# daniestevez/gr4-packet-modem

Hardware: AMD Instinct MI355X
Metric: RX Msamples/s (syncword-detect + RRC chain) (higher is better)
Workload: dtype f32; 1 GPU; configs[1]: 1 channel/GPU, full RX front end (SyncwordDetection 9 bins FFT 2048 + tag gate + CFC + 32-arm RRC SymbolFilter + wipe-off + Costas) on resident burst+AWGN stream; channels_per_gpu=1, freq_bins=9, parallelism=channel-per-gpu x1, input=generated on each GPU, pipelined_streams=4, pipeline_driver=native (gr4pm_packet_receiver), windows=2, correlator_lookahead=2

## Files before the change

### gr4-packet-modem_amd/_abi.py

```python
import ctypes as C
import os

import numpy as np

_HERE = os.path.dirname(os.path.abspath(__file__))
LIB_PATH = os.environ.get("GR4PM_LIB") or os.path.join(_HERE, "libgr4pm_hip.so")

OK = 0
INSUFFICIENT_INPUT_ITEMS = 1
INSUFFICIENT_OUTPUT_ITEMS = 2
TAG_SYNCWORD = 1
TAG_OTHER = 2

TAG_DTYPE = np.dtype(
    [
        ("index", "<u8"),
        ("amplitude", "<f4"),
        ("phase", "<f4"),
        ("freq", "<f8"),
        ("freq_bin", "<i4"),
        ("noise_power", "<f4"),
        ("esn0_db", "<f4"),
        ("time_est", "<f4"),
        ("flags", "<i4"),
# ... 298 lines not shown
    "gr4pm_iq_unpack", "gr4pm_iq_pack",
    "gr4pm_ddc_taps", "gr4pm_ddc_create", "gr4pm_ddc_destroy", "gr4pm_ddc_reset", "gr4pm_ddc_output_items",
    "gr4pm_ddc_frequencies", "gr4pm_ddc_process", "gr4pm_ddc_process_iq",
    "gr4pm_ddc_rational_taps", "gr4pm_ddc_create_rational", "gr4pm_ddc_extract", "gr4pm_ddc_extract_iq",
    "gr4pm_duc_taps", "gr4pm_duc_create", "gr4pm_duc_destroy", "gr4pm_duc_reset", "gr4pm_duc_output_items",
    "gr4pm_duc_frequencies", "gr4pm_duc_process",
    "gr4pm_duc_rational_taps", "gr4pm_duc_create_rational",
    "gr4pm_spectrum_window", "gr4pm_spectrum_float_run", "gr4pm_spectrum_create", "gr4pm_spectrum_destroy",
    "gr4pm_spectrum_reset", "gr4pm_spectrum_process", "gr4pm_spectrum_process_iq", "gr4pm_spectrum_read",
    "gr4pm_find_carriers",
    "gr4pm_spectrogram_create", "gr4pm_spectrogram_destroy", "gr4pm_spectrogram_reset", "gr4pm_spectrogram_rows",
    "gr4pm_spectrogram_process", "gr4pm_spectrogram_process_iq", "gr4pm_spectrogram_band_power", "gr4pm_find_bursts",
    "gr4pm_line_spectrum_float_run", "gr4pm_line_spectrum_create", "gr4pm_line_spectrum_destroy", "gr4pm_line_spectrum_process",
    "gr4pm_find_line", "gr4pm_simplest_ratio",
    "gr4pm_row_resampler_taps", "gr4pm_row_resampler_create", "gr4pm_row_resampler_destroy",
    "gr4pm_row_resampler_output_lengths", "gr4pm_row_resampler_tile_items", "gr4pm_row_resampler_process",
]

_lib = None


class Gr4pmError(RuntimeError):
    """what the reference raises as gr::exception"""


def lib():
    global _lib
    if _lib is not None:
        return _lib
    if not os.path.exists(LIB_PATH):
        raise ImportError(
            f"{LIB_PATH} is missing: build it with `python -c 'import __graft_entry__ as g; g.build()'` "
            "(hipcc --offload-arch=gfx950). There is no CPU fallback.")
    try:
        import torch
    except ImportError:
        pass
    L = C.CDLL(LIB_PATH)
    vp, sz, szp = C.c_void_p, C.c_size_t, C.POINTER(C.c_size_t)
    L.gr4pm_last_error.restype = C.c_char_p
    L.gr4pm_version.restype = C.c_char_p
    L.gr4pm_device_count.restype = C.c_int
    if hasattr(L, "gr4pm_test_fail_allocations"):
        L.gr4pm_test_fail_allocations.argtypes = [C.c_long, C.c_long]
        L.gr4pm_test_fail_allocations.restype = None
        L.gr4pm_test_allocation_count.restype = C.c_ulonglong
    L.gr4pm_syncword_detection_create.argtypes = [C.POINTER(SyncwordDetectionParams), C.POINTER(vp)]
    L.gr4pm_syncword_detection_destroy.argtypes = [vp]
    L.gr4pm_syncword_detection_destroy.restype = None
    L.gr4pm_syncword_detection_reset.argtypes = [vp]
    L.gr4pm_syncword_detection_syncword_samples_size.argtypes = [vp]
    L.gr4pm_syncword_detection_syncword_samples_size.restype = sz
    L.gr4pm_syncword_detection_self_corr.argtypes = [vp]
    L.gr4pm_syncword_detection_self_corr.restype = C.c_float
    L.gr4pm_syncword_detection_items_consumed.argtypes = [vp]
    L.gr4pm_syncword_detection_items_consumed.restype = C.c_uint64
    L.gr4pm_syncword_detection_scan_counts.argtypes = [vp, sz, C.POINTER(C.c_uint64), C.POINTER(C.c_uint64)]
    L.gr4pm_syncword_detection_scan_counts.restype = None
    L.gr4pm_syncword_detection_process.argtypes = [vp, vp, sz, sz, vp, sz, szp, vp, sz, vp]
    L.gr4pm_syncword_detection_last_zpow.argtypes = [vp, vp, sz]
    L.gr4pm_syncword_detection_correlate_only.argtypes = [vp, vp, sz, sz]
    L.gr4pm_syncword_detection_hint_next.argtypes = [vp, vp, sz, sz]
    L.gr4pm_syncword_detection_announce.argtypes = [vp, vp, sz, sz]
    L.gr4pm_syncword_detection_filter_create.argtypes = [C.POINTER(SdfParams), C.POINTER(vp)]
    L.gr4pm_syncword_detection_filter_destroy.argtypes = [vp]
    L.gr4pm_syncword_detection_filter_destroy.restype = None
    L.gr4pm_syncword_detection_filter_reset.argtypes = [vp]
    L.gr4pm_syncword_detection_filter_process.argtypes = [vp, vp, sz, vp, sz, C.c_int, vp, sz, sz, szp, szp, szp,
                                                          C.POINTER(C.c_int)]
    L.gr4pm_syncword_detection_filter_gate.argtypes = [vp, vp, sz, vp, sz, C.c_int, vp, szp]
    L.gr4pm_rotator_create.argtypes = [C.POINTER(RotatorParams), C.POINTER(vp)]
    L.gr4pm_rotator_destroy.argtypes = [vp]
    L.gr4pm_rotator_destroy.restype = None
    L.gr4pm_rotator_reset.argtypes = [vp]
    L.gr4pm_rotator_process.argtypes = [vp, vp, sz, sz, vp, vp, vp, sz]
    L.gr4pm_costas_loop_create.argtypes = [C.POINTER(CostasParams), C.POINTER(vp)]
    L.gr4pm_costas_loop_destroy.argtypes = [vp]
    L.gr4pm_costas_loop_destroy.restype = None
    L.gr4pm_costas_loop_reset.argtypes = [vp]
    L.gr4pm_costas_loop_coeffs.argtypes = [vp, C.POINTER(C.c_float), C.POINTER(C.c_float)]
    L.gr4pm_costas_loop_coeffs.restype = None
    L.gr4pm_costas_loop_set.argtypes = [vp, C.c_double, C.c_int]
    L.gr4pm_costas_loop_process.argtypes = [vp, vp, sz, sz, vp, vp, vp, sz]
    L.gr4pm_syncword_wipeoff_create.argtypes = [C.POINTER(WipeoffParams), C.POINTER(vp)]
    L.gr4pm_syncword_wipeoff_destroy.argtypes = [vp]
    L.gr4pm_syncword_wipeoff_destroy.restype = None
    L.gr4pm_syncword_wipeoff_reset.argtypes = [vp]
    L.gr4pm_syncword_wipeoff_process.argtypes = [vp, vp, sz, vp, vp, sz]
    L.gr4pm_syncword_wipeoff_process_channels.argtypes = [vp, sz, vp, sz, vp, vp, vp]
    L.gr4pm_cfc_symbol_filter_run_channels.argtypes = [vp, C.c_int, vp, sz, vp, sz, sz, vp, sz, vp, vp, vp, sz, vp, vp, vp, sz, sz]
    L.gr4pm_multichannel_receiver_set_input_in_place.argtypes = [vp, C.c_int]
    L.gr4pm_interp_fir_create.argtypes = [C.POINTER(InterpFirParams), C.POINTER(vp)]
    L.gr4pm_interp_fir_destroy.argtypes = [vp]
    L.gr4pm_interp_fir_destroy.restype = None
    L.gr4pm_interp_fir_reset.argtypes = [vp]
    L.gr4pm_interp_fir_process.argtypes = [vp, vp, sz, vp]
    L.gr4pm_symbol_filter_create.argtypes = [C.POINTER(SymbolFilterParams), C.POINTER(vp)]
    L.gr4pm_symbol_filter_destroy.argtypes = [vp]
    L.gr4pm_symbol_filter_destroy.restype = None
    L.gr4pm_symbol_filter_reset.argtypes = [vp]
    L.gr4pm_symbol_filter_process.argtypes = [vp, vp, sz, vp, sz, vp, sz, vp, sz, szp, szp, szp]
    L.gr4pm_cfc_symbol_filter_process.argtypes = [vp, vp, vp, sz, vp, sz, vp, sz, vp, sz, szp, szp, szp]
    L.gr4pm_cfc_symbol_filter_plan.argtypes = [vp, sz, vp, sz, C.POINTER(C.c_int)]
    L.gr4pm_cfc_symbol_filter_run.argtypes = [vp, C.c_int, vp, vp, sz, vp, sz, vp, sz, vp, sz, szp, szp, szp]
    L.gr4pm_pfb_arb_resampler_create.argtypes = [C.POINTER(PfbArbParams), C.POINTER(vp)]
    L.gr4pm_pfb_arb_resampler_destroy.argtypes = [vp]
    L.gr4pm_pfb_arb_resampler_destroy.restype = None
    L.gr4pm_pfb_arb_resampler_reset.argtypes = [vp]
    L.gr4pm_pfb_arb_resampler_process.argtypes = [vp, vp, sz, vp, sz, szp, szp]
    L.gr4pm_payload_metadata_insert_create.argtypes = [C.POINTER(PmiParams), C.POINTER(vp)]
    L.gr4pm_payload_metadata_insert_destroy.argtypes = [vp]
    L.gr4pm_payload_metadata_insert_destroy.restype = None
    L.gr4pm_payload_metadata_insert_reset.argtypes = [vp]
    L.gr4pm_payload_metadata_insert_process.argtypes = [vp, vp, sz, vp, sz, vp, sz, vp, sz, C.c_int, vp, sz,
                                                        szp, szp, szp, szp, szp]
    L.gr4pm_costas_loop_process_packets.argtypes = [vp, vp, sz, vp, vp, sz]
    L.gr4pm_syncword_detection_filter_gate_resolve.argtypes = [vp, vp]
    L.gr4pm_payload_metadata_insert_resolve.argtypes = [vp, vp]
    L.gr4pm_syncword_remove_create.argtypes = [C.POINTER(SyncwordRemoveParams), C.POINTER(vp)]
    L.gr4pm_syncword_remove_destroy.argtypes = [vp]
    L.gr4pm_syncword_remove_destroy.restype = None
    L.gr4pm_syncword_remove_reset.argtypes = [vp]
    L.gr4pm_syncword_remove_process.argtypes = [vp, vp, sz, vp, vp, sz, vp, sz, szp, szp]
    L.gr4pm_constellation_llr_decoder_create.argtypes = [C.POINTER(LlrParams), C.POINTER(vp)]
    L.gr4pm_constellation_llr_decoder_destroy.argtypes = [vp]
    L.gr4pm_constellation_llr_decoder_destroy.restype = None
    L.gr4pm_constellation_llr_decoder_process.argtypes = [vp, vp, sz, vp, sz, vp, sz, vp, sz, szp, szp]
    L.gr4pm_additive_scrambler_create.argtypes = [C.POINTER(ScramblerParams), C.POINTER(vp)]
    L.gr4pm_additive_scrambler_destroy.argtypes = [vp]
    L.gr4pm_additive_scrambler_destroy.restype = None
    L.gr4pm_additive_scrambler_reset.argtypes = [vp]
    L.gr4pm_additive_scrambler_process.argtypes = [vp, vp, sz, vp, vp, sz]
    L.gr4pm_header_payload_split_create.argtypes = [C.POINTER(HeaderPayloadSplitParams), C.POINTER(vp)]
    L.gr4pm_header_payload_split_destroy.argtypes = [vp]
    L.gr4pm_header_payload_split_destroy.restype = None
    L.gr4pm_header_payload_split_reset.argtypes = [vp]
    L.gr4pm_header_payload_split_process.argtypes = [vp, vp, sz, vp, szp, vp, szp, vp, sz, vp, szp, vp, szp, sz]
    L.gr4pm_header_payload_split_process_c64.argtypes = [vp, vp, sz, vp, szp, vp, szp, vp, sz, vp, szp, vp, szp, sz]
    L.gr4pm_header_fec_decoder_create.argtypes = [C.POINTER(HeaderFecDecoderParams), C.POINTER(vp)]
    L.gr4pm_header_fec_decoder_destroy.argtypes = [vp]
    L.gr4pm_header_fec_decoder_destroy.restype = None
    L.gr4pm_header_fec_decoder_process.argtypes = [vp, vp, sz, vp, vp]
    L.gr4pm_header_parse.argtypes = [vp, vp, sz, vp, vp]
    L.gr4pm_header_parse.restype = None
    L.gr4pm_binary_slicer_process.argtypes = [vp, sz, vp, C.c_int, vp]
    L.gr4pm_pack_bits_process.argtypes = [vp, sz, vp, sz, C.c_uint, C.c_int, vp]
    L.gr4pm_slice_pack_process.argtypes = [vp, sz, vp, vp]
    L.gr4pm_crc_check_create.argtypes = [C.POINTER(CrcCheckParams), C.POINTER(vp)]
    L.gr4pm_crc_check_destroy.argtypes = [vp]
    L.gr4pm_crc_check_destroy.restype = None
    L.gr4pm_crc_check_compute.argtypes = [vp, vp, sz]
    L.gr4pm_crc_check_compute.restype = C.c_uint64
    L.gr4pm_crc_check_process.argtypes = [vp, vp, vp, vp, sz, vp, vp, szp]
    L.gr4pm_mapper_process.argtypes = [vp, sz, vp, vp, sz, C.c_int, vp]
    L.gr4pm_burst_shaper_process.argtypes = [vp, sz, vp, C.c_int, vp, sz, vp, sz, vp, vp, sz, vp]
    L.gr4pm_packet_receiver_create.argtypes = [C.POINTER(PacketReceiverParams), C.POINTER(vp)]
    L.gr4pm_packet_receiver_destroy.argtypes = [vp]
    L.gr4pm_packet_receiver_destroy.restype = None
    L.gr4pm_packet_receiver_submit.argtypes = [vp, vp, sz, vp, vp, sz, C.c_uint64, vp, sz, vp, sz, vp, sz]
    L.gr4pm_packet_receiver_announce.argtypes = [vp, vp, sz]
    L.gr4pm_multichannel_receiver_create.argtypes = [C.POINTER(MultiChannelReceiverParams), C.POINTER(vp)]
    L.gr4pm_multichannel_receiver_destroy.argtypes = [vp]
    L.gr4pm_multichannel_receiver_destroy.restype = None
    L.gr4pm_multichannel_receiver_announce.argtypes = [vp, vp, sz, sz]
    L.gr4pm_multichannel_receiver_process.argtypes = [vp, vp, sz, sz, C.c_uint64, vp, sz, szp, szp, vp, szp, vp, szp]
    L.gr4pm_multichannel_receiver_submit.argtypes = [vp, vp, sz, sz, C.c_uint64, vp, sz, szp]
# ... 115 lines not shown
```

### gr4-packet-modem_amd/csrc/costas_loop.hip

```cpp
#include "stream_blocks.hpp"
#include "hostlogic/costas_plan.hpp"

namespace gr4pm {
namespace {

struct CostasState {
    float phase, freq;
};
using hostlogic::CostasSeg;

__device__ __forceinline__ void sincosf_glibc(float y, float* s_out, float* c_out)
{
    const double hpi_inv = 0x1.45F306DC9C883p+23, hpi = 0x1.921FB54442D18p0;
    const double C0 = 0x1p0, C1 = -0x1.ffffffd0c621cp-2, C2 = 0x1.55553e1068f19p-5, C3 = -0x1.6c087e89a359dp-10,
                 C4 = 0x1.99343027bf8c3p-16, S1 = -0x1.555545995a603p-3, S2 = 0x1.1107605230bc4p-7,
                 S3 = -0x1.994eb3774cf24p-13;
    const double x0 = static_cast<double>(y);
    const int n = (static_cast<int>(x0 * hpi_inv) + 0x800000) >> 24;
    const double x = fma(-static_cast<double>(n), hpi, x0);
    const double x2 = x * x;
    const double x3 = x * x2;
    const double s1 = fma(x2, S3, S2);
    const double x7 = x3 * x2;
    const double sp = fma(x7, s1, fma(x3, S1, x));
    const double x4 = x2 * x2;
    const double c2 = fma(x2, C4, C3);
    const double c1 = fma(x2, C1, C0);
    const double x6 = x4 * x2;
    const double cp = fma(x6, c2, fma(x4, C2, c1));
    float sn = static_cast<float>(sp), cs = static_cast<float>(cp);
    const unsigned sb = __builtin_amdgcn_bitop3_b32(0x7fffffffu, __float_as_uint(sn), static_cast<unsigned>(__double2hiint(x)), 0xca);
    const unsigned cb = __float_as_uint(cs);
    const unsigned swap = static_cast<unsigned>(__builtin_amdgcn_sbfe(n, 0, 1));
    const unsigned s0 = __builtin_amdgcn_bitop3_b32(swap, cb, sb, 0xca);
    const unsigned c0 = __builtin_amdgcn_bitop3_b32(swap, sb, cb, 0xca);
    const unsigned q = static_cast<unsigned>(n) << 30;
    *s_out = __uint_as_float(__builtin_amdgcn_bitop3_b32(s0, q, 0x80000000u, 0x78));
    *c_out = __uint_as_float(__builtin_amdgcn_bitop3_b32(c0, q + 0x40000000u, 0x80000000u, 0x78));
}

__device__ __forceinline__ float costas_wrap(float phase, float pi_f)
{
    const float K = 0x1p100f, two_pi = 2.0f * pi_f;
    const float pi_below = __uint_as_float(__float_as_uint(pi_f) - 1u);
    float up, down;
    asm("v_fma_f32 %0, %2, %3, -%4 clamp\n\t"
        "v_fma_f32 %1, -%2, %3, -%5 clamp"
        : "=&v"(up), "=&v"(down)
        : "v"(phase), "v"(K), "v"(pi_below * K), "v"(pi_f * K));
    return __builtin_fmaf(up - down, -two_pi, phase);
}

template <int CONSTELLATION>
__device__ __forceinline__ cf costas_step(cf x, float& phase, float& freq, float k1, float k2)
{
    const float pi_f = 3.14159265358979323846f;
    float sn, cs;
#ifdef GR4PM_COSTAS_HW_SINCOS
    sn = __sinf(phase);
    cs = __cosf(phase);
#else
    sincosf_glibc(phase, &sn, &cs);
#endif
    const cf lo = { cs, -sn };
    const cf z = cmul(x, lo);
    float error;
    if constexpr (CONSTELLATION == 0) error = z.y;
    else if constexpr (CONSTELLATION == 1) error = z.x * z.y;
    else error = (z.x > 0 ? z.y : -z.y) + (z.y > 0 ? -z.x : z.x);
    freq += k2 * error;
    phase += k1 * error + freq;
    phase = costas_wrap(phase, pi_f);
    return z;
}

template <int CONSTELLATION, int KV = 8>
__device__ __forceinline__ void costas_run(const cf* __restrict__ in, cf* __restrict__ out, size_t base,
                                           unsigned len, float& phase, float& freq, float k1, float k2)
{
    auto step = [&](cf x) -> cf { return costas_step<CONSTELLATION>(x, phase, freq, k1, k2); };
    constexpr int kV = KV;
    constexpr unsigned kC = 2 * kV;
    unsigned j = 0;
    if (((base + j) & 1) && j < len) {
        out[base + j] = step(in[base + j]);
        ++j;
    }
    const unsigned n_chunks = (len - j) / kC;
    if (n_chunks > 0) {
        const float4* ip = reinterpret_cast<const float4*>(in + base + j);
        float4* op = reinterpret_cast<float4*>(out + base + j);
        float4 a[kV], b[kV];
        auto load = [&](float4(&v)[kV], unsigned c) {
            const float4* p = ip + static_cast<size_t>(min(c, n_chunks - 1)) * kV;
#pragma unroll
            for (int u = 0; u < kV; ++u) v[u] = p[u];
            asm volatile("" : "+v"(phase), "+v"(freq) : : "memory");
        };
        auto run = [&](float4(&v)[kV], unsigned c) {
#pragma unroll
            for (int u = 0; u < kV; ++u) {
                const cf z0 = step(cf{ v[u].x, v[u].y });
                const cf z1 = step(cf{ v[u].z, v[u].w });
                v[u] = make_float4(z0.x, z0.y, z1.x, z1.y);
            }
            float4* q = op + static_cast<size_t>(c) * kV;
#pragma unroll
            for (int u = 0; u < kV; ++u) q[u] = v[u];
        };
        load(a, 0);
        unsigned c = 0;
        for (; c + 2 <= n_chunks; c += 2) {
            load(b, c + 1);
            run(a, c);
            load(a, c + 2);
            run(b, c + 1);
        }
        if (c < n_chunks) run(a, c);
        j += n_chunks * kC;
    }
    for (; j < len; ++j) out[base + j] = step(in[base + j]);
}

template <int CONSTELLATION, int KV = 8>
__global__ void k_costas(const CostasSeg* __restrict__ segs, unsigned n_segs,
                         const CostasState* __restrict__ state, CostasState* __restrict__ state_next,
                         float k1, float k2,
                         const cf* __restrict__ in, cf* __restrict__ out, size_t stride)
{
    const unsigned s = blockIdx.x * blockDim.x + threadIdx.x;
    if (s >= n_segs) return;
    __builtin_amdgcn_s_setprio(GR4PM_SERIAL_PRIO);
    const CostasSeg g = segs[s];
    float phase, freq;
    if (g.mode == 0) {
        phase = state[g.channel].phase;
        freq = state[g.channel].freq;
    } else {
        phase = g.phase0;
        freq = 0.0f;
    }
    costas_run<CONSTELLATION, KV>(in, out, static_cast<size_t>(g.channel) * stride + g.start, g.len, phase, freq, k1,
                              k2);
    if (g.last) {
        state_next[g.channel].phase = phase;
        state_next[g.channel].freq = freq;
    }
}

template <int CONSTELLATION, int KV>
__global__ __attribute__((amdgpu_num_vgpr(16))) void k_costas_cap(const CostasSeg* __restrict__ segs, unsigned n_segs,
                                                               const CostasState* __restrict__ state,
                                                               CostasState* __restrict__ state_next, float k1, float k2,
                                                               const cf* __restrict__ in, cf* __restrict__ out,
                                                               size_t stride)
{
    const unsigned s = blockIdx.x * blockDim.x + threadIdx.x;
    if (s >= n_segs) return;
    __builtin_amdgcn_s_setprio(GR4PM_SERIAL_PRIO);
    const CostasSeg g = segs[s];
    float phase, freq;
    if (g.mode == 0) {
        phase = state[g.channel].phase;
        freq = state[g.channel].freq;
    } else {
        phase = g.phase0;
        freq = 0.0f;
    }
    costas_run<CONSTELLATION, KV>(in, out, static_cast<size_t>(g.channel) * stride + g.start, g.len, phase, freq, k1, k2);
    if (g.last) {
        state_next[g.channel].phase = phase;
        state_next[g.channel].freq = freq;
    }
}

using hostlogic::CostasChain;
using hostlogic::CostasPiece;
template <int KV>
__device__ __forceinline__ void costas_chains_body(const CostasChain* __restrict__ chains, unsigned n_chains,
                                                   const CostasPiece* __restrict__ pieces,
                                                   const CostasState* __restrict__ state,
                                                   CostasState* __restrict__ state_next, const cf* __restrict__ in,
                                                   cf* __restrict__ out)
{
    const unsigned s = blockIdx.x * blockDim.x + threadIdx.x;
    if (s >= n_chains) return;
    __builtin_amdgcn_s_setprio(GR4PM_SERIAL_PRIO);
    const CostasChain ch = chains[s];
    float phase, freq;
    if (ch.mode == 0) {
        phase = state[0].phase;
        freq = state[0].freq;
    } else {
        phase = ch.phase0;
        freq = 0.0f;
    }
    for (unsigned q = 0; q < ch.n_pieces; ++q) {
        const CostasPiece pc = pieces[ch.piece0 + q];
        const cf* src = in + pc.in_off;
        if (pc.constellation == 0) costas_run<0, KV>(src, out, pc.start, pc.len, phase, freq, pc.k1, pc.k2);
        else if (pc.constellation == 1) costas_run<1, KV>(src, out, pc.start, pc.len, phase, freq, pc.k1, pc.k2);
        else costas_run<2, KV>(src, out, pc.start, pc.len, phase, freq, pc.k1, pc.k2);
    }
    if (ch.last) {
        state_next[0].phase = phase;
        state_next[0].freq = freq;
    }
}
template <int KV>
__global__ void k_costas_chains(const CostasChain* __restrict__ chains, unsigned n_chains,
                                const CostasPiece* __restrict__ pieces, const CostasState* __restrict__ state,
                                CostasState* __restrict__ state_next, const cf* __restrict__ in,
                                cf* __restrict__ out)
{
    costas_chains_body<KV>(chains, n_chains, pieces, state, state_next, in, out);
}
__global__ __attribute__((amdgpu_num_vgpr(16))) void k_costas_chains_cap(const CostasChain* __restrict__ chains, unsigned n_chains,
                                                                      const CostasPiece* __restrict__ pieces,
                                                                      const CostasState* __restrict__ state,
                                                                      CostasState* __restrict__ state_next,
                                                                      const cf* __restrict__ in, cf* __restrict__ out)
{
    costas_chains_body<2>(chains, n_chains, pieces, state, state_next, in, out);
}

__global__ void k_sincosf(const float* __restrict__ x, size_t n, float* __restrict__ sn, float* __restrict__ cs)
{
    const size_t i = static_cast<size_t>(blockIdx.x) * blockDim.x + threadIdx.x;
    if (i < n) sincosf_glibc(x[i], sn + i, cs + i);
}

__global__ void k_costas_wrap(const float* __restrict__ x, size_t n, float* __restrict__ out)
{
    const size_t i = static_cast<size_t>(blockIdx.x) * blockDim.x + threadIdx.x;
    if (i < n) out[i] = costas_wrap(x[i], 3.14159265358979323846f);
}

#ifdef GR4PM_EXPERIMENTS
__global__ __launch_bounds__(64) void k_serial_fake(unsigned ticks, float* sink)
{
    const unsigned long long t0 = wall_clock64();
    float x = threadIdx.x;
    while (wall_clock64() - t0 < ticks) {
#pragma unroll
        for (int i = 0; i < 32; ++i) x = __builtin_fmaf(x, 1.0001f, 0.5f);
    }
    if (x == 12345.0f) *sink = x;
}
#endif

}
}

using namespace gr4pm;

struct gr4pm_costas_loop : gr4pm::hostlogic::CostasHostState {
    size_t n_channels;
    hipStream_t stream;
    DevBuf<CostasState> state;
    int st_cur = 0;
    int small_footprint = 0;
    DevBuf<CostasSeg> segs;
    DevBuf<CostasChain> chains;
    DevBuf<CostasPiece> pieces;
};
using hostlogic::costas_coeffs;

extern "C" {

gr4pm_status gr4pm_costas_loop_create(const gr4pm_costas_loop_params* p, gr4pm_costas_loop** out)
try {
    if (!p || !out || p->n_channels == 0 || p->constellation < 0 || p->constellation > 2)
        return GR4PM_ERR_INVALID;
    *out = nullptr;
    GR4PM_TRY(require_device());
    std::unique_ptr<gr4pm_costas_loop> h(new (std::nothrow) gr4pm_costas_loop);
    if (!h) return GR4PM_ERR_NOMEM;
    h->loop_bandwidth = p->loop_bandwidth;
    h->constellation = p->constellation;
    h->n_channels = p->n_channels;
    h->stream = static_cast<hipStream_t>(p->stream);
    costas_coeffs(*h);
    GR4PM_TRY(h->state.alloc(2 * h->n_channels));
    GR4PM_TRY(h->state.zero(h->stream));
    static const char* form = gr4pm::experiment_env("GR4PM_COSTAS_FORM", false);
    if (form) h->small_footprint = std::min(2, std::max(0, atoi(form)));
    return finish_create(h, out, "costas_loop");
}
GR4PM_ABI_CATCH
void gr4pm_costas_loop_destroy(gr4pm_costas_loop* h)
try {
    if (!h) return;
    (void)hipStreamSynchronize(h->stream);
    delete h;
}
GR4PM_ABI_CATCH_VOID
gr4pm_status gr4pm_costas_loop_reset(gr4pm_costas_loop* h)
try {
    if (!h) return GR4PM_ERR_INVALID;
    GR4PM_TRY(h->state.zero(h->stream));
    GR4PM_HIP_TRY(hipStreamSynchronize(h->stream));
    h->st_cur = 0;
    return GR4PM_OK;
}
GR4PM_ABI_CATCH
void gr4pm_costas_loop_coeffs(const gr4pm_costas_loop* h, float* k1, float* k2)
try {
    *k1 = h->k1;
    *k2 = h->k2;
}
GR4PM_ABI_CATCH_VOID
gr4pm_status gr4pm_costas_loop_set(gr4pm_costas_loop* h, double loop_bandwidth, int constellation)
try {
    if (!h || constellation < 0 || constellation > 2) return GR4PM_ERR_INVALID;
    h->loop_bandwidth = loop_bandwidth;
    h->constellation = constellation;
    costas_coeffs(*h);
    return GR4PM_OK;
}
GR4PM_ABI_CATCH

extern "C++" {
template <typename NOf>
static gr4pm_status costas_process_impl(gr4pm_costas_loop* h, const gr4pm_c64* in, size_t stride, NOf n_of,
                                        gr4pm_c64* out, const gr4pm_tag* tags, const uint32_t* tag_channel,
                                        size_t n_tags)
{
    static const bool costas_no_sort = gr4pm::experiment_env("GR4PM_COSTAS_NO_SORT", false) != nullptr;
    std::vector<CostasSeg> segs;
    hostlogic::costas_segments(h->n_channels, n_of, tags, tag_channel, n_tags, costas_no_sort, segs);
    hipStream_t s = h->stream;
    GR4PM_TRY(upload_vec(h->segs, segs, s));
    if (timing_skip("seg_stats")) {
        size_t longest = 0, total = 0;
        for (const auto& g : segs) longest = std::max<size_t>(longest, g.len), total += g.len;
        fprintf(stderr, "[gr4pm costas] %zu segments, %zu items, longest %zu\n", segs.size(), total, longest);
    }
    static const unsigned wg = gr4pm::experiment_env_wg("GR4PM_COSTAS_WG", 64u, 1u, 1024u);
    const dim3 grid(grid_for(segs.size(), wg)), block(wg);
    const unsigned n_segs = static_cast<unsigned>(segs.size());
    const CostasState* st_in = h->state.p + h->st_cur * h->n_channels;
    CostasState* st_out = h->state.p + (h->st_cur ^ 1) * h->n_channels;
    h->st_cur ^= 1;
    auto launch = [&](auto kernel) {
#ifdef GR4PM_EXPERIMENTS
        if (timing_skip("costas_fake")) {
            unsigned wgs = grid.x, ticks = 83000u, lds = 0u;
            static const char* fake = gr4pm::experiment_env("GR4PM_FAKE", true);
            if (fake) sscanf(fake, "%u,%u,%u", &wgs, &ticks, &lds);
            wgs = std::max(wgs, 1u);
            if (lds > 48 * 1024)
                (void)hipFuncSetAttribute(reinterpret_cast<const void*>(k_serial_fake),
                                          hipFuncAttributeMaxDynamicSharedMemorySize, static_cast<int>(lds));
            hipLaunchKernelGGL(k_serial_fake, dim3(wgs), block, lds, s, ticks, reinterpret_cast<float*>(st_out));
            return;
        }
#endif
        if (timing_skip("costas")) return;
        hipLaunchKernelGGL(kernel, grid, block, 0, s, h->segs.p, n_segs, st_in, st_out, h->k1, h->k2,
                           reinterpret_cast<const cf*>(in), reinterpret_cast<cf*>(out), stride);
    };
    size_t call_symbols = 0;
    for (const auto& g : segs) call_symbols += g.len;
    static const char* cap_min = gr4pm::experiment_env("GR4PM_COSTAS_CAP_MIN_LOG2", false);
    const size_t cap_from = size_t{ 1 } << (cap_min ? std::min(40, std::max(0, atoi(cap_min))) : 25);
    if (h->small_footprint >= 2 && call_symbols >= cap_from) {
        if (h->constellation == 0) launch(k_costas_cap<0, 2>);
        else if (h->constellation == 1) launch(k_costas_cap<1, 2>);
        else launch(k_costas_cap<2, 2>);
    } else if (h->small_footprint == 1) {
        if (h->constellation == 0) launch(k_costas<0, 2>);
        else if (h->constellation == 1) launch(k_costas<1, 2>);
        else launch(k_costas<2, 2>);
    } else {
        if (h->constellation == 0) launch(k_costas<0, 8>);
        else if (h->constellation == 1) launch(k_costas<1, 8>);
        else launch(k_costas<2, 8>);
    }
    GR4PM_HIP_TRY(hipGetLastError());
    GR4PM_HIP_TRY(final_sync(s));
    return GR4PM_OK;
}
}

gr4pm_status gr4pm_costas_loop_set_small_footprint(gr4pm_costas_loop* h, int on)
try {
    if (!h) return GR4PM_ERR_INVALID;
    h->small_footprint = on < 0 ? 0 : (on > 2 ? 2 : on);
    return GR4PM_OK;
}
GR4PM_ABI_CATCH

gr4pm_status gr4pm_costas_loop_process(gr4pm_costas_loop* h, const gr4pm_c64* in, size_t stride, size_t n,
                                       gr4pm_c64* out, const gr4pm_tag* tags, const uint32_t* tag_channel,
                                       size_t n_tags)
try {
    if (!h) return GR4PM_ERR_INVALID;
    if (n == 0) return GR4PM_OK;
    if (!in || !out) {
        set_error("null sample pointer");
        return GR4PM_ERR_INVALID;
    }
    return costas_process_impl(h, in, stride, [n](size_t) { return n; }, out, tags, tag_channel, n_tags);
}
GR4PM_ABI_CATCH

gr4pm_status gr4pm_costas_loop_process_ragged(gr4pm_costas_loop* h, const gr4pm_c64* in, size_t stride,
                                              const size_t* n_per_channel, gr4pm_c64* out, const gr4pm_tag* tags,
                                              const uint32_t* tag_channel, size_t n_tags)
try {
    if (!h || !n_per_channel) return GR4PM_ERR_INVALID;
    if (!in || !out) {
        set_error("null sample pointer");
        return GR4PM_ERR_INVALID;
    }
    return costas_process_impl(h, in, stride, [n_per_channel](size_t c) { return n_per_channel[c]; }, out, tags,
                               tag_channel, n_tags);
}
GR4PM_ABI_CATCH

gr4pm_status gr4pm_costas_loop_process_packets(gr4pm_costas_loop* h, const gr4pm_c64* in, size_t n,
                                               gr4pm_c64* out, const gr4pm_packet_tag* tags, size_t n_tags)
try {
    return gr4pm::costas_loop_process_packets_from(h, in, nullptr, 0, n, out, tags, n_tags);
}
GR4PM_ABI_CATCH

}

gr4pm_status gr4pm::costas_loop_process_packets_from(gr4pm_costas_loop* h, const gr4pm_c64* in, const hostlogic::CopySpan* spans,
                                                     size_t n_spans, size_t n, gr4pm_c64* out, const gr4pm_packet_tag* tags,
                                                     size_t n_tags)
{
    if (!h) return GR4PM_ERR_INVALID;
    if (h->n_channels != 1) {
        set_error("process_packets needs a single-channel CostasLoop");
        return GR4PM_ERR_INVALID;
    }
    if (n == 0) return GR4PM_OK;
    if (!in || !out) {
        set_error("null sample pointer");
        return GR4PM_ERR_INVALID;
    }
    std::vector<CostasChain> chains;
    std::vector<CostasPiece> pieces;
    GR4PM_TRY(hostlogic::costas_packet_chains(*h, spans, n_spans, n, tags, n_tags, chains, pieces));
    if (chains.empty()) return GR4PM_OK;
    hipStream_t s = h->stream;
    GR4PM_TRY(upload_vec(h->chains, chains, s));
    GR4PM_TRY(upload_vec(h->pieces, pieces, s));
    if (!timing_skip("costas_chains")) {
        static const char* cap_min = gr4pm::experiment_env("GR4PM_COSTAS_CAP_MIN_LOG2", false);
        const size_t cap_from = size_t{ 1 } << (cap_min ? std::min(40, std::max(0, atoi(cap_min))) : 25);
        auto launch = [&](auto kernel) {
            hipLaunchKernelGGL(kernel, dim3(grid_for(chains.size(), 64)), dim3(64), 0, s, h->chains.p,
                               static_cast<unsigned>(chains.size()), h->pieces.p, h->state.p + h->st_cur,
                               h->state.p + (h->st_cur ^ 1), reinterpret_cast<const cf*>(in), reinterpret_cast<cf*>(out));
        };
        if (h->small_footprint >= 2 && n >= cap_from) launch(k_costas_chains_cap);
        else if (h->small_footprint == 1) launch(k_costas_chains<2>);
        else launch(k_costas_chains<8>);
    }
    h->st_cur ^= 1;
    GR4PM_HIP_TRY(hipGetLastError());
    GR4PM_HIP_TRY(final_sync(s));
    return GR4PM_OK;
}

extern "C" {

gr4pm_status gr4pm_sincosf(const float* x, size_t n, float* sin_out, float* cos_out)
// ... 26 lines not shown
```

### gr4-packet-modem_amd/csrc/multichannel_receiver.hip

```cpp
#include <algorithm>
#include <chrono>
#include <cmath>
#include <cstdio>
#include <cstdlib>
#include <condition_variable>
#include <cstring>
#include <deque>
#include <memory>
#include <mutex>
#include <thread>
#include <vector>

#include "common.hpp"
#include "hostlogic/slot_queue.hpp"

using namespace gr4pm;

constexpr int kMcSlots = 4;

struct gr4pm_multichannel_receiver {
    gr4pm_multichannel_receiver_params p{};
    int device = 0;
    gr4pm_syncword_detection* sd = nullptr;
    hipStream_t sd_stream = nullptr;
// ... 237 lines not shown
            s.status = exception_status(which == 1 ? "multichannel receiver, stage 1"
                                                   : which == 2 ? "multichannel receiver, stage 2" : "multichannel receiver, stage 3");
            std::strncpy(s.error, gr4pm_last_error(), sizeof(s.error) - 1);
            if (which == 3) s.t_done = std::chrono::steady_clock::now();
        });
}

extern "C" {

gr4pm_status gr4pm_multichannel_receiver_create(const gr4pm_multichannel_receiver_params* p,
                                                gr4pm_multichannel_receiver** out)
try {
    if (!p || !out || p->n_channels == 0 || p->samples_per_symbol == 0 || p->max_items < 2048) return GR4PM_ERR_INVALID;
    *out = nullptr;
    GR4PM_TRY(require_device());
    auto* h = new (std::nothrow) gr4pm_multichannel_receiver;
    if (!h) return GR4PM_ERR_NOMEM;
    h->p = *p;
    h->p.tags_cap = std::max<size_t>(p->tags_cap, 64);
    auto bail = [&](gr4pm_status st) {
        gr4pm_multichannel_receiver_destroy(h);
        return st;
    };
    const unsigned n_workers = static_cast<unsigned>(std::min<size_t>(std::max(p->workers, 1), p->n_channels));
    int least = 0, greatest = 0;
    if (hipDeviceGetStreamPriorityRange(&least, &greatest) != hipSuccess) return bail(GR4PM_ERR_HIP);
    if (hipStreamCreateWithPriority(&h->sd_stream, hipStreamNonBlocking, greatest) != hipSuccess) return bail(GR4PM_ERR_HIP);
    h->streams.assign(n_workers, nullptr);
    for (unsigned w = 0; w < n_workers; ++w) {
        const int prio = w % 3 == 0 ? 0 : (w % 3 == 1 ? greatest : least);
        if (hipStreamCreateWithPriority(&h->streams[w], hipStreamNonBlocking, prio) != hipSuccess) return bail(GR4PM_ERR_HIP);
    }
    const size_t sps = p->samples_per_symbol;
    std::vector<float> rrc(((sps * 11) | 1));
    const size_t n_rrc = gr4pm_firdes_root_raised_cosine(1.0, static_cast<double>(sps), 1.0, 0.35, sps * 11, rrc.data());
    if (n_rrc == 0) return bail(GR4PM_ERR_NOMEM);
    rrc.resize(n_rrc);
    float norm = 0.0f;
    for (float v : rrc) norm += v * v;
    norm = std::sqrt(norm);
    for (float& v : rrc) v /= norm;
    static const uint8_t syncword[64] = {
        0, 0, 0, 0, 0, 0, 1, 1, 0, 1, 0, 0, 0, 1, 1, 1, 0, 1, 1, 1, 0, 1, 1, 0, 1, 1, 0, 0, 0, 1, 1, 1,
        0, 0, 1, 0, 0, 1, 1, 1, 0, 0, 1, 0, 1, 0, 0, 0, 1, 0, 0, 1, 0, 1, 0, 1, 1, 0, 1, 1, 0, 0, 0, 0 };
    const gr4pm_c64 bpsk[2] = { { 1.0f, 0.0f }, { -1.0f, 0.0f } };
    gr4pm_syncword_detection_params sp{};
    sp.fft_size = 2048;
    sp.samples_per_symbol = sps;
    sp.rrc_taps = rrc.data();
    sp.n_rrc_taps = rrc.size();
    sp.syncword = syncword;
    sp.n_syncword = 64;
    sp.constellation = bpsk;
    sp.n_constellation = 2;
    sp.min_freq_bin = -p->syncword_freq_bins;
    sp.max_freq_bin = p->syncword_freq_bins;
    sp.time_threshold = 768;
    sp.power_threshold = p->syncword_threshold;
    sp.n_channels = p->n_channels;
    sp.max_items = p->max_items;
    sp.stream = h->sd_stream;
    gr4pm_status st = gr4pm_syncword_detection_create(&sp, &h->sd);
    if (st != GR4PM_OK) return bail(st);
    gr4pm::sd_set_coresident(h->sd, true);
    const size_t arms = 32;
    std::vector<float> pfb(((arms * sps * 11) | 1));
    const size_t n_pfb = gr4pm_firdes_root_raised_cosine(static_cast<double>(arms) / static_cast<double>(norm),
                                                         static_cast<double>(arms * sps), 1.0, 0.35, arms * sps * 11,
                                                         pfb.data());
    if (n_pfb == 0) return bail(GR4PM_ERR_NOMEM);
    pfb.resize(n_pfb - 1);
    float bipolar[64];
    for (int i = 0; i < 64; ++i) bipolar[i] = syncword[i] ? -1.0f : 1.0f;
    h->chains.reset(new (std::nothrow) gr4pm_multichannel_receiver::Chain[p->n_channels]);
    if (!h->chains) return bail(GR4PM_ERR_NOMEM);
    if (hipStreamCreateWithPriority(&h->batch_stream, hipStreamNonBlocking, greatest) != hipSuccess) return bail(GR4PM_ERR_HIP);
    gr4pm_rotator_params rp{ 1, 0.0f, (rrc.size() - 1) / 2 + sps, p->n_channels, h->batch_stream };
    if ((st = gr4pm_rotator_create(&rp, &h->cfc)) != GR4PM_OK) return bail(st);
    if (hipStreamCreateWithPriority(&h->costas_stream, hipStreamNonBlocking, least) != hipSuccess) return bail(GR4PM_ERR_HIP);
    gr4pm_costas_loop_params cp{ 0.01, p->costas_constellation, p->n_channels, h->costas_stream };
    if ((st = gr4pm_costas_loop_create(&cp, &h->costas)) != GR4PM_OK) return bail(st);
    {
        static const char* small = gr4pm::experiment_env("GR4PM_COSTAS_SMALL", false);
        if (small) (void)gr4pm_costas_loop_set_small_footprint(h->costas, atoi(small));
    }
    for (size_t c = 0; c < p->n_channels; ++c) {
        auto& ch = h->chains[c];
        hipStream_t s = h->streams[c % n_workers];
        gr4pm_syncword_detection_filter_params fp{ sps, 64, 128, s };
        if ((st = gr4pm_syncword_detection_filter_create(&fp, &ch.sdf)) != GR4PM_OK) return bail(st);
        gr4pm_symbol_filter_params fsp{ sps, pfb.data(), pfb.size(), arms, rrc.size() - 1, 0, s };
        if ((st = gr4pm_symbol_filter_create(&fsp, &ch.symf)) != GR4PM_OK) return bail(st);
        gr4pm_syncword_wipeoff_params wp{ bipolar, 64, s };
        if ((st = gr4pm_syncword_wipeoff_create(&wp, &ch.wipe)) != GR4PM_OK) return bail(st);
    }
    {
        const char* e = getenv("GR4PM_MC_PER_CHANNEL");
        h->per_channel_launches = e && e[0] == '1';
        const size_t C = p->n_channels;
        h->v_symf.resize(C);
        h->v_wipe.resize(C);
        for (size_t c = 0; c < C; ++c) {
            h->v_symf[c] = h->chains[c].symf;
            h->v_wipe[c] = h->chains[c].wipe;
        }
        h->v_tags_in.assign(C, nullptr);
        h->v_tags_out.assign(C, nullptr);
        h->v_n_tags_in.assign(C, 0);
        h->v_n_tags_out.assign(C, 0);
        h->v_produced.assign(C, 0);
    }
    h->hist = 2 * 768 + 1;
    h->sd_fft = sp.fft_size;
    h->sd_stride = sp.fft_size - (63 * sps + rrc.size()) + 1;
    for (auto& t : h->tails) {
        if ((st = t.alloc(h->hist * p->n_channels)) != GR4PM_OK) return bail(st);
        if ((st = t.zero(h->sd_stream)) != GR4PM_OK) return bail(st);
    }
    if (hipStreamSynchronize(h->sd_stream) != hipSuccess) return bail(GR4PM_ERR_HIP);
    h->y_stride = (p->max_items + 63) & ~size_t{ 63 };
    for (auto& sl : h->slots) {
        if ((st = sl.y.alloc(h->y_stride * p->n_channels)) != GR4PM_OK) return bail(st);
        sl.det_tags.resize(p->n_channels * h->p.tags_cap);
        sl.n_det.assign(p->n_channels, 0);
        sl.produced.assign(p->n_channels, 0);
        sl.ch.resize(p->n_channels);
        for (auto& cb : sl.ch) {
            cb.tags.resize(h->p.tags_cap);
            cb.sym_tags.resize(h->p.tags_cap + 64);
        }
    }
    if (hipGetDevice(&h->device) != hipSuccess) return bail(GR4PM_ERR_HIP);
    try {
        h->workers.reserve(n_workers);
        for (unsigned w = 0; w < n_workers; ++w) h->workers.emplace_back([h, w] { h->worker(w); });
        h->t_stage1 = std::thread([h] { h->stage_loop(1); });
        h->t_stage2 = std::thread([h] { h->stage_loop(2); });
        h->t_stage3 = std::thread([h] { h->stage_loop(3); });
    } catch (...) {
        return bail(exception_status("gr4pm_multichannel_receiver_create (threads)"));
    }
    *out = h;
    return GR4PM_OK;
}
GR4PM_ABI_CATCH

void gr4pm_multichannel_receiver_destroy(gr4pm_multichannel_receiver* h)
try {
    if (!h) return;
    {
        std::lock_guard<std::mutex> l(h->m);
        h->quit = true;
    }
    h->cv_go.notify_all();
    h->to_stage1.stop();
    h->to_stage2.stop();
    h->to_stage3.stop();
    h->done.stop();
    for (std::thread* t : { &h->t_stage1, &h->t_stage2, &h->t_stage3 })
        if (t->joinable()) t->join();
    for (auto& t : h->workers)
        if (t.joinable()) t.join();
    gr4pm_syncword_detection_destroy(h->sd);
    for (size_t c = 0; h->chains && c < h->p.n_channels; ++c) {
        auto& ch = h->chains[c];
        gr4pm_syncword_detection_filter_destroy(ch.sdf);
        gr4pm_symbol_filter_destroy(ch.symf);
// ... 156 lines not shown
```

Measured before the change: 67550 Msamples/s.

## Add LDS ring-buffered async-load Costas kernel and make it the receiver default

Adds a Costas loop kernel in which each lane streams its segment through an 8-slot LDS ring filled with global_load_lds_dwordx4 direct-to-LDS loads. Several chunks are kept in flight so the serial per-symbol phase recursion no longer stalls on global memory latency. The multichannel receiver now sets small_footprint=2 by default, which picks the ring kernel when the wavefront fits within the CU count and the call is large enough. Other changes: the wrap constants move to SGPR operands, VGPRs are capped at 16, and an unaligned head or tail symbol is handled separately. The risks are extra LDS usage, tight register pressure, and a default switch of kernel path for large calls.

```diff
diff --git a/gr4-packet-modem_amd/_abi.py b/gr4-packet-modem_amd/_abi.py
--- a/gr4-packet-modem_amd/_abi.py
+++ b/gr4-packet-modem_amd/_abi.py
@@ -404,6 +404,8 @@
     L.gr4pm_costas_loop_coeffs.restype = None
     L.gr4pm_costas_loop_set.argtypes = [vp, C.c_double, C.c_int]
     L.gr4pm_costas_loop_process.argtypes = [vp, vp, sz, sz, vp, vp, vp, sz]
+    L.gr4pm_costas_loop_process_ragged.argtypes = [vp, vp, sz, szp, vp, vp, vp, sz]
+    L.gr4pm_costas_loop_set_small_footprint.argtypes = [vp, C.c_int]
     L.gr4pm_syncword_wipeoff_create.argtypes = [C.POINTER(WipeoffParams), C.POINTER(vp)]
     L.gr4pm_syncword_wipeoff_destroy.argtypes = [vp]
     L.gr4pm_syncword_wipeoff_destroy.restype = None
diff --git a/gr4-packet-modem_amd/csrc/costas_loop.hip b/gr4-packet-modem_amd/csrc/costas_loop.hip
--- a/gr4-packet-modem_amd/csrc/costas_loop.hip
+++ b/gr4-packet-modem_amd/csrc/costas_loop.hip
@@ -1,5 +1,6 @@
 #include "stream_blocks.hpp"
 #include "hostlogic/costas_plan.hpp"
+#include "hostlogic/costas_ring_plan.hpp"
 
 namespace gr4pm {
 namespace {
@@ -47,7 +48,7 @@
     asm("v_fma_f32 %0, %2, %3, -%4 clamp\n\t"
         "v_fma_f32 %1, -%2, %3, -%5 clamp"
         : "=&v"(up), "=&v"(down)
-        : "v"(phase), "v"(K), "v"(pi_below * K), "v"(pi_f * K));
+        : "v"(phase), "v"(K), "s"(pi_below * K), "s"(pi_f * K));
     return __builtin_fmaf(up - down, -two_pi, phase);
 }
 
@@ -174,6 +175,88 @@
     }
 }
 
+__device__ __forceinline__ void ring_dma(const float4* src, uint32_t slot_base)
+{
+    asm volatile("s_mov_b32 m0, %1\n\ts_nop 0\n\tglobal_load_lds_dwordx4 %0, off" : : "v"(src), "s"(slot_base) : "memory");
+}
+template <unsigned VMCNT>
+__device__ __forceinline__ void ring_wait()
+{
+    asm volatile("s_waitcnt vmcnt(%c0) lgkmcnt(0)" : : "i"(VMCNT) : "memory");
+}
+
+template <int CONSTELLATION>
+__global__ __attribute__((amdgpu_num_vgpr(16))) void k_costas_ring(
+    const CostasSeg* __restrict__ segs, unsigned n_segs, const CostasState* __restrict__ state,
+    CostasState* __restrict__ state_next, float k1, float k2, const cf* __restrict__ in, cf* __restrict__ out, size_t stride)
+{
+    using namespace hostlogic;
+    __shared__ float4 ring[kCostasRingSlots * 64];
+    static_assert(sizeof(ring) == kCostasRingSlots * kCostasRingSlotBytes, "one slot = 64 lanes x 16 bytes");
+    const unsigned lane = threadIdx.x;
+    const unsigned s = blockIdx.x * 64u + lane;
+    __builtin_amdgcn_s_setprio(GR4PM_SERIAL_PRIO);
+    CostasSeg g{};
+    g.mode = 1;
+    if (s < n_segs) g = segs[s];
+    float phase, freq;
+    if (g.mode == 0) {
+        phase = state[g.channel].phase;
+        freq = state[g.channel].freq;
+    } else {
+        phase = g.phase0;
+        freq = 0.0f;
+    }
+    auto step = [&](cf x) -> cf { return costas_step<CONSTELLATION>(x, phase, freq, k1, k2); };
+    const size_t base = static_cast<size_t>(g.channel) * stride + g.start;
+    const CostasRingLane rl = costas_ring_lane(base, g.len);
+    const unsigned n_chunks = rl.n_chunks;
+    const uint32_t ring_base = static_cast<uint32_t>(reinterpret_cast<uintptr_t>((__attribute__((address_space(3))) char*)ring));
+    size_t q = (base + rl.head) >> 1;
+    auto request = [&](unsigned r) {
+        asm volatile("" : "+v"(q));
+        ring_dma(reinterpret_cast<const float4*>(in) + q + costas_ring_request_chunk(r, n_chunks),
+                 ring_base + costas_ring_slot(r) * kCostasRingSlotBytes);
+    };
+    const bool asks = n_chunks > 0;
+    asm volatile("" : "+v"(phase), "+v"(freq));
+    if (asks) {
+#pragma unroll
+        for (unsigned r = 0; r < kCostasRingPrologue; ++r) request(r);
+    }
+    if (rl.head) out[base] = step(in[base]);
+    auto iteration = [&](unsigned c, auto vmcnt) {
+        ring_wait<decltype(vmcnt)::value>();
+        const float4 v = ring[costas_ring_slot(c) * 64u + lane];
+        if (asks) request(costas_ring_request_of_iteration(c));
+        if (c < n_chunks) {
+            const cf z0 = step(cf{ v.x, v.y });
+            const cf z1 = step(cf{ v.z, v.w });
+            asm volatile("" : "+v"(q));
+            reinterpret_cast<float4*>(out)[q + c] = make_float4(z0.x, z0.y, z1.x, z1.y);
+        }
+    };
+    static_assert(kCostasRingWaitFill == costas_ring_wait(0) && kCostasRingWaitFill == costas_ring_wait(kCostasRingPrologue - 1) &&
+                      kCostasRingWaitSteady == costas_ring_wait(kCostasRingPrologue),
+                  "the two immediates are the schedule's");
+    unsigned c = 0;
+    for (; c < kCostasRingPrologue && __builtin_amdgcn_ballot_w64(c < n_chunks) != 0; ++c)
+        iteration(c, std::integral_constant<unsigned, kCostasRingWaitFill>{});
+    for (; __builtin_amdgcn_ballot_w64(c < n_chunks) != 0; ++c)
+        iteration(c, std::integral_constant<unsigned, kCostasRingWaitSteady>{});
+    asm volatile("s_waitcnt vmcnt(0)" ::: "memory");
+    unsigned s_again = s;
+    asm volatile("" : "+v"(s_again));
+    CostasSeg e{};
+    if (s_again < n_segs) e = segs[s_again];
+    const size_t end = static_cast<size_t>(e.channel) * stride + e.start + e.len;
+    if (costas_ring_lane(end - e.len, e.len).tail) out[end - 1] = step(in[end - 1]);
+    if (e.last) {
+        state_next[e.channel].phase = phase;
+        state_next[e.channel].freq = freq;
+    }
+}
+
 using hostlogic::CostasChain;
 using hostlogic::CostasPiece;
 template <int KV>
@@ -260,6 +343,7 @@
     DevBuf<CostasState> state;
     int st_cur = 0;
     int small_footprint = 0;
+    int n_cus = 0;
     DevBuf<CostasSeg> segs;
     DevBuf<CostasChain> chains;
     DevBuf<CostasPiece> pieces;
@@ -284,7 +368,10 @@
     GR4PM_TRY(h->state.alloc(2 * h->n_channels));
     GR4PM_TRY(h->state.zero(h->stream));
     static const char* form = gr4pm::experiment_env("GR4PM_COSTAS_FORM", false);
-    if (form) h->small_footprint = std::min(2, std::max(0, atoi(form)));
+    if (form) h->small_footprint = std::min(3, std::max(0, atoi(form)));
+    int dev = 0;
+    hipDeviceProp_t prop;
+    if (hipGetDevice(&dev) == hipSuccess && hipGetDeviceProperties(&prop, dev) == hipSuccess) h->n_cus = prop.multiProcessorCount;
     return finish_create(h, out, "costas_loop");
 }
 GR4PM_ABI_CATCH
@@ -362,9 +449,14 @@
     };
     size_t call_symbols = 0;
     for (const auto& g : segs) call_symbols += g.len;
-    static const char* cap_min = gr4pm::experiment_env("GR4PM_COSTAS_CAP_MIN_LOG2", false);
+    const char* cap_min = gr4pm::experiment_env("GR4PM_COSTAS_CAP_MIN_LOG2", false);
     const size_t cap_from = size_t{ 1 } << (cap_min ? std::min(40, std::max(0, atoi(cap_min))) : 25);
-    if (h->small_footprint >= 2 && call_symbols >= cap_from) {
+    const bool ring = h->small_footprint == 2 && wg == 64u && grid.x <= static_cast<unsigned>(std::max(h->n_cus, 0));
+    if (ring && call_symbols >= cap_from) {
+        if (h->constellation == 0) launch(k_costas_ring<0>);
+        else if (h->constellation == 1) launch(k_costas_ring<1>);
+        else launch(k_costas_ring<2>);
+    } else if (h->small_footprint >= 2 && call_symbols >= cap_from) {
         if (h->constellation == 0) launch(k_costas_cap<0, 2>);
         else if (h->constellation == 1) launch(k_costas_cap<1, 2>);
         else launch(k_costas_cap<2, 2>);
@@ -386,7 +478,7 @@
 gr4pm_status gr4pm_costas_loop_set_small_footprint(gr4pm_costas_loop* h, int on)
 try {
     if (!h) return GR4PM_ERR_INVALID;
-    h->small_footprint = on < 0 ? 0 : (on > 2 ? 2 : on);
+    h->small_footprint = on < 0 ? 0 : (on > 3 ? 3 : on);
     return GR4PM_OK;
 }
 GR4PM_ABI_CATCH
diff --git a/gr4-packet-modem_amd/csrc/hostlogic/costas_ring_plan.hpp b/gr4-packet-modem_amd/csrc/hostlogic/costas_ring_plan.hpp
--- /dev/null
+++ b/gr4-packet-modem_amd/csrc/hostlogic/costas_ring_plan.hpp
@@ -0,0 +1,48 @@
+#pragma once
+
+#if defined(__HIPCC__)
+#define GR4PM_RING_HD __host__ __device__
+#else
+#define GR4PM_RING_HD
+#endif
+
+namespace gr4pm {
+namespace hostlogic {
+
+constexpr unsigned kCostasRingSlots = 8;
+constexpr unsigned kCostasRingSlotBytes = 1024;
+constexpr unsigned kCostasRingChunkSymbols = 2;
+constexpr unsigned kCostasRingPrologue = kCostasRingSlots - 1;
+static_assert((kCostasRingSlots & (kCostasRingSlots - 1)) == 0 && kCostasRingSlots >= 2, "slot = chunk & (slots - 1)");
+
+struct CostasRingLane {
+    unsigned head;
+    unsigned n_chunks;
+    unsigned tail;
+};
+
+GR4PM_RING_HD constexpr CostasRingLane costas_ring_lane(unsigned long long base, unsigned len)
+{
+    CostasRingLane l{};
+    l.head = (base & 1ull) && len > 0 ? 1u : 0u;
+    l.n_chunks = (len - l.head) / kCostasRingChunkSymbols;
+    l.tail = len - l.head - l.n_chunks * kCostasRingChunkSymbols;
+    return l;
+}
+
+GR4PM_RING_HD constexpr unsigned costas_ring_request_chunk(unsigned r, unsigned n_chunks)
+{
+    return r < n_chunks - 1 ? r : n_chunks - 1;
+}
+GR4PM_RING_HD constexpr unsigned costas_ring_slot(unsigned r) { return r & (kCostasRingSlots - 1); }
+GR4PM_RING_HD constexpr unsigned costas_ring_request_of_iteration(unsigned c) { return c + kCostasRingPrologue; }
+
+constexpr unsigned kCostasRingWaitFill = kCostasRingSlots - 2;
+constexpr unsigned kCostasRingWaitSteady = (kCostasRingSlots - 2) + (kCostasRingSlots - 1);
+GR4PM_RING_HD constexpr unsigned costas_ring_wait(unsigned c)
+{
+    return c < kCostasRingSlots - 1 ? kCostasRingWaitFill : kCostasRingWaitSteady;
+}
+
+}
+}
diff --git a/gr4-packet-modem_amd/csrc/multichannel_receiver.hip b/gr4-packet-modem_amd/csrc/multichannel_receiver.hip
--- a/gr4-packet-modem_amd/csrc/multichannel_receiver.hip
+++ b/gr4-packet-modem_amd/csrc/multichannel_receiver.hip
@@ -343,7 +343,7 @@
     if ((st = gr4pm_costas_loop_create(&cp, &h->costas)) != GR4PM_OK) return bail(st);
     {
         static const char* small = gr4pm::experiment_env("GR4PM_COSTAS_SMALL", false);
-        if (small) (void)gr4pm_costas_loop_set_small_footprint(h->costas, atoi(small));
+        (void)gr4pm_costas_loop_set_small_footprint(h->costas, small ? atoi(small) : 2);
     }
     for (size_t c = 0; c < p->n_channels; ++c) {
         auto& ch = h->chains[c];
```

Measured after the change: 66090 Msamples/s. -2.2%, worse.
